# Westlake-AI/SemiReward

Measured on AMD Instinct MI355X. Metric: unlabeled images/sec/node (FlexMatch+SR, ViT-S CIFAR-100), higher is better.
Workload: dtype bf16

## Files before the change

### include/srhip.h

```cpp
#ifndef SRHIP_H
#define SRHIP_H

#ifdef __cplusplus
extern "C" {
#endif

enum {
  SRHIP_EPI_BF16 = 0,
  SRHIP_EPI_GELU_BF16 = 1,
  SRHIP_EPI_RESID_F32 = 2,
  SRHIP_EPI_DGELU_BF16 = 3,
  SRHIP_EPI_F32 = 4
};
int srhip_gemm_nt(int epilogue, const void* A, int lda, const void* B, int ldb, void* C, int ldc, int M, int N, int K,
                  const float* bias, const float* row_scale, int rows_per_sample, const void* aux_in, void* aux_out,
                  int ldaux, float alpha, float beta, void* stream);
#define SRHIP_GEMM_PLAN_TILE128 0
#define SRHIP_GEMM_PLAN_SMALL64 1
#define SRHIP_GEMM_PLAN_BIG256 2
#define SRHIP_GEMM_PLAN_BIG128 3
#define SRHIP_GEMM_PLAN_BIG2WG 4
#define SRHIP_GEMM_PLAN_PP256 5
int srhip_gemm_nt_plan(int epilogue, int M, int N, int K, float beta);
int srhip_gemm_nt_planned(int epilogue, const void* A, int lda, const void* B, int ldb, void* C, int ldc, int M, int N, int K,
// ... 22 lines not shown
#define SRHIP_TN_OVERWRITE 2
typedef struct srhip_group_tn_desc {
  const void* A; const void* B; float* C; float* dbias;
  int M, N, K, lda, ldb, ldc, tile_start, flags;
} srhip_group_tn_desc;
int srhip_gemm_tn_grouped_f32(const srhip_group_tn_desc* desc_dev, int n_problems, int total_tiles, float alpha, float beta,
                              void* stream);
typedef struct srhip_slab_desc {
  float* dst; const float* src; long long stride;
  int count, n_slabs, block_start, pad0;
} srhip_slab_desc;
int srhip_slab_reduce_f32(const srhip_slab_desc* desc_dev, int n, int total_blocks, void* stream);
int srhip_gemm_tn_grouped_pp_f32(const srhip_group_tn_desc* desc_dev, int n_problems, int total_tiles, float alpha, float beta,
                                 void* stream);

int srhip_attn_fwd(const void* qkv, void* out, float* lse, int B, int N, int H, float scale, void* stream);
int srhip_attn_bwd(const void* qkv, const void* out, const void* d_out, const float* lse, void* dqkv, float* delta_ws,
                   int B, int N, int H, float scale, void* stream);

int srhip_attn_masked_fwd(const void* qkv, void* out, float* lse, const int* key_len, int B, int N, int H, float scale,
                          unsigned drop_key, unsigned drop_thresh, float drop_scale, void* stream);
int srhip_attn_masked_bwd(const void* qkv, const void* out, const void* d_out, const float* lse, void* dqkv, float* delta_ws,
                          const int* key_len, int B, int N, int H, float scale, unsigned drop_key, unsigned drop_thresh,
                          float drop_scale, void* stream);

int srhip_layernorm_fwd(const float* x, const float* gamma, const float* beta, float eps, void* out, float* mean,
                        float* rstd, int M, int D, void* stream);
int srhip_layernorm_bwd(const void* dy, const float* x, const float* mean, const float* rstd, const float* gamma,
                        float* dx, float* dgamma, float* dbeta, int M, int D, void* stream);
int srhip_layernorm_bwd_cast(const void* dy, const float* x, const float* mean, const float* rstd, const float* gamma, float* dx, float* dgamma,
                             float* dbeta, void* out_bf16, const float* row_scale, int rows_per_sample, int M, int D, void* stream);
int srhip_layernorm_bwd_part(const void* dy, const float* x, const float* mean, const float* rstd, const float* gamma, float* dx, float* part,
                             int n_rep, void* out_bf16, const float* row_scale, int rows_per_sample, int M, int D, void* stream);
typedef struct srhip_ln_reduce_desc { float* dgamma; float* dbeta; } srhip_ln_reduce_desc;
int srhip_ln_grad_reduce(const srhip_ln_reduce_desc* desc_dev, float* part, int n_ln, int n_rep, int D, void* stream);
typedef struct srhip_dw_tail {
  const srhip_ln_reduce_desc* ln_desc; float* ln_part;
  const float* dlogits; const float* feat; float* dWh; float* dbh;
  const float* dx; const float* img; const int* img_index; float* dpos; float* dcls; float* pe_ws;
  int n_ln, n_rep, C, B, D, in_chans, HW, ps;
} srhip_dw_tail;
int srhip_gemm_tn_grouped_tail_f32(const srhip_group_tn_desc* desc_dev, int n_problems, int total_tiles, float alpha, float beta,
                                   const srhip_dw_tail* tail, void* stream);
int srhip_patch_embed_bwd_fold(const float* ws, float* dWp, float* dbp, int B, int C, int HW, int ps, int D, void* stream);

int srhip_mlp_fused(const float* x, float* x_out, const float* ln_gamma, const float* ln_beta, float eps, const void* W1,
                    const float* b1, const void* W2, const float* b2, const float* row_scale, int rows_per_sample, int save_rows,
                    void* save_ln2, void* save_pre, void* save_h, float* save_mean, float* save_rstd, int M, int D, int Hd,
                    void* stream);
int srhip_gelu_eval(const float* x, float* y_erf, float* y_poly, int n, void* stream);
int srhip_mlp_fused_proj(const float* x, float* x_out, const void* ao, const void* Wp, const float* bp, const float* row_scale1,
                         int ao_scaled, const float* ln_gamma, const float* ln_beta, float eps, const void* W1, const float* b1, const void* W2,
                         const float* b2, const float* row_scale2, int rows_per_sample, void* ln_next, const float* next_gamma,
                         const float* next_beta, int M, int D, int Hd, void* stream);

int srhip_attn_block_supported(int N, int D, int H);
int srhip_attn_block_fused(const void* xn_bf16, const void* Wqkv, const float* bqkv, const void* qkv_extra, void* out, const float* out_scale,
                           int B, int N, int D, int H, float scale, void* stream);

int srhip_patch_embed_fwd(const float* img, const int* img_index, const float* Wp, const float* bp, const float* cls,
                          const float* pos, float* x, int B, int C, int HW, int ps, int D, void* stream);
int srhip_patch_embed_bwd(const float* dx, const float* img, const int* img_index, float* dWp, float* dbp, float* dcls,
                          float* dpos, int B, int C, int HW, int ps, int D, void* stream);
long srhip_patch_embed_bwd_ws_floats(int B, int C, int HW, int ps, int D);
int srhip_patch_embed_bwd_ws(const float* dx, const float* img, const int* img_index, float* dWp, float* dbp, float* dcls,
                             float* dpos, float* ws, int B, int C, int HW, int ps, int D, void* stream);
// ... 272 lines not shown
```

### semireward_amd/_lib.py

```python
import ctypes
import os
from ctypes import c_double, c_float, c_int, c_long, c_longlong, c_uint, c_ulonglong, c_void_p

import torch

HERE = os.path.dirname(os.path.abspath(__file__))
LIB_PATH = os.path.join(HERE, "libsrhip.so")

EPI_BF16, EPI_GELU_BF16, EPI_RESID_F32, EPI_DGELU_BF16, EPI_F32 = range(5)
X3_EPI_F32, X3_EPI_GELU_F32, X3_EPI_RESID_F32 = range(3)
X3B_NT, X3B_NN = range(2)
X3B_EPI_F32, X3B_EPI_ACC, X3B_EPI_DGELU, X3B_EPI_GELU_PRE = range(4)
REDUCE_NONE, REDUCE_MEAN, REDUCE_SUM = range(3)

P, I, F, L, Dbl, U = c_void_p, c_int, c_float, c_long, c_double, c_uint
SIGNATURES = {
    "srhip_gemm_nt": (I, [I, P, I, P, I, P, I, I, I, I, P, P, I, P, P, I, F, F, P]),
    "srhip_gemm_nt_plan": (I, [I, I, I, I, F]),
    "srhip_gemm_nt_planned": (I, [I, P, I, P, I, P, I, I, I, I, P, P, I, P, P, I, F, F, I, P]),
    "srhip_vit_fork": (I, [P, P, P, I, I, I, I, P]),
    "srhip_vit_fanout": (I, [P, P, I, P, P, I, P, P, c_longlong, I, I, P]),
    "srhip_gemm_small_max_grid": (I, [I]),
    "srhip_gemm_nt_grouped_f32": (I, [P, I, I, F, F, P]),
    "srhip_gemm_nt_grouped_n64_f32": (I, [P, I, I, F, F, P]),
    "srhip_gemm_tn_grouped_f32": (I, [P, I, I, F, F, P]),
    "srhip_gemm_tn_grouped_pp_f32": (I, [P, I, I, F, F, P]),
    "srhip_gemm_tn_grouped_tail_f32": (I, [P, I, I, F, F, P, P]),
    "srhip_patch_embed_bwd_fold": (I, [P, P, P, I, I, I, I, I, P]),
    "srhip_slab_reduce_f32": (I, [P, I, I, P]),
    "srhip_attn_fwd": (I, [P, P, P, I, I, I, F, P]),
    "srhip_attn_bwd": (I, [P, P, P, P, P, P, I, I, I, F, P]),
    "srhip_layernorm_fwd": (I, [P, P, P, F, P, P, P, I, I, P]),
    "srhip_layernorm_bwd": (I, [P, P, P, P, P, P, P, P, I, I, P]),
    "srhip_layernorm_bwd_cast": (I, [P, P, P, P, P, P, P, P, P, P, I, I, I, P]),
    "srhip_layernorm_bwd_part": (I, [P, P, P, P, P, P, P, I, P, P, I, I, I, P]),
    "srhip_ln_grad_reduce": (I, [P, P, I, I, I, P]),
    "srhip_mlp_fused": (I, [P, P, P, P, F, P, P, P, P, P, I, I, P, P, P, P, P, I, I, I, P]),
    "srhip_attn_block_supported": (I, [I, I, I]),
    "srhip_attn_block_fused": (I, [P, P, P, P, P, P, I, I, I, I, F, P]),
    "srhip_gelu_eval": (I, [P, P, P, I, P]),
    "srhip_mlp_fused_proj": (I, [P, P, P, P, P, P, I, P, P, F, P, P, P, P, P, I, P, P, P, I, I, I, P]),
    "srhip_adam_bias_corrections": (I, [F, F, I, P]),
    "srhip_adamw_flat_dyn": (I, [P, P, P, P, P, P, P, I, P, P, P, F, F, F, Dbl, F, P, I, P]),
    "srhip_adam_flat_dyn": (I, [P, P, P, P, L, F, F, F, F, P, P]),
    "srhip_droppath_fill_cols_dyn": (I, [P, P, P, I, I, I, P, c_ulonglong, P]),
    "srhip_patch_embed_fwd": (I, [P, P, P, P, P, P, P, I, I, I, I, I, P]),
    "srhip_patch_embed_bwd": (I, [P, P, P, P, P, P, P, I, I, I, I, I, P]),
    "srhip_patch_embed_bwd_ws_floats": (L, [I, I, I, I, I]),
    "srhip_patch_embed_bwd_ws": (I, [P, P, P, P, P, P, P, P, I, I, I, I, I, P]),
    "srhip_patch_im2col": (I, [P, P, P, I, I, I, I, P]),
    "srhip_patch_assemble": (I, [P, P, P, P, P, I, I, I, P]),
    "srhip_patch_grad_operands": (I, [P, P, P, P, I, I, I, P]),
    "srhip_gemm_nt_x3": (I, [I, P, I, P, I, P, I, I, I, I, P, P, I, P]),
    "srhip_attn_fwd_x3": (I, [P, P, I, I, I, F, P]),
    "srhip_layernorm_fwd_f32": (I, [P, P, P, F, P, P, P, I, I, P]),
    "srhip_patch_im2col_f32": (I, [P, P, P, I, I, I, I, P]),
    "srhip_attn_fwd_x3_lse": (I, [P, P, P, I, I, I, F, P]),
    "srhip_gemm_x3": (I, [I, I, P, I, P, I, P, I, I, I, I, P, P, P, I, P]),
    "srhip_gemm_tn_x3_grouped": (I, [P, I, I, P]),
    "srhip_attn_bwd_x3": (I, [P, P, P, P, P, P, I, I, I, F, P]),
    "srhip_layernorm_bwd_part_f32": (I, [P, P, P, P, P, P, P, I, P, P, I, I, I, P]),
    "srhip_patch_grad_operands_f32": (I, [P, P, P, P, I, I, I, P]),
    "srhip_scale_rows_f32": (I, [P, P, I, P, L, I, P]),
    "srhip_cls_head_fwd": (I, [P, P, P, F, P, P, P, P, P, P, I, I, I, I, P]),
    "srhip_cls_head_fwd_scatter": (I, [P, P, P, F, P, P, P, P, P, P, P, P, P, I, I, I, I, P]),
    "srhip_cls_head_bwd": (I, [P, P, P, P, P, P, P, P, P, P, P, I, I, I, I, P]),
    "srhip_cast_scale_rows": (I, [P, P, I, P, L, I, P]),
    "srhip_transpose_to_bf16": (I, [P, I, I, P, I, I, I, I, I, P, P]),
# ... 136 lines not shown
```

### semireward_amd/csrc/vit_ops.hip

```cpp
#include "common.h"
#include "srhip.h"
#include "tail_ops.h"

namespace {

template <int NV, typename TOUT = bf16_t>
__global__ __launch_bounds__(256) void ln_fwd_kernel(const float* __restrict__ x, const float* __restrict__ gamma,
                                                    const float* __restrict__ beta, float eps, TOUT* __restrict__ out,
                                                    float* __restrict__ mean, float* __restrict__ rstd, int M) {
  constexpr int D = NV * 128, RW = 2;
  const int row0 = (blockIdx.x * 4 + (threadIdx.x >> 6)) * RW, lane = threadIdx.x & 63;
  if (row0 >= M) return;
  float2 v[RW][NV], g[NV], b[NV];
#pragma unroll
  for (int r = 0; r < RW; ++r) {
    const float2* xr = reinterpret_cast<const float2*>(x + (size_t)min(row0 + r, M - 1) * D);
#pragma unroll
    for (int i = 0; i < NV; ++i) v[r][i] = xr[i * 64 + lane];
  }
#pragma unroll
  for (int i = 0; i < NV; ++i) {
    g[i] = reinterpret_cast<const float2*>(gamma)[i * 64 + lane];
    b[i] = reinterpret_cast<const float2*>(beta)[i * 64 + lane];
  }
#pragma unroll
  for (int r = 0; r < RW; ++r) {
    const int row = row0 + r;
    if (row >= M) break;
    float s = 0.f;
#pragma unroll
    for (int i = 0; i < NV; ++i) s += v[r][i].x + v[r][i].y;
    const float mu = wave_sum(s) * (1.0f / D);
    float q = 0.f;
// ... 1 lines not shown
    for (int i = 0; i < NV; ++i) { const float a = v[r][i].x - mu, c = v[r][i].y - mu; q += a * a + c * c; }
    const float rs = rsqrtf(wave_sum(q) * (1.0f / D) + eps);
    if constexpr (sizeof(TOUT) == 4) {
      float2* orow = reinterpret_cast<float2*>(out + (size_t)row * D);
#pragma unroll
      for (int i = 0; i < NV; ++i)
        orow[i * 64 + lane] = make_float2((v[r][i].x - mu) * rs * g[i].x + b[i].x, (v[r][i].y - mu) * rs * g[i].y + b[i].y);
    } else {
      uint32_t* orow = reinterpret_cast<uint32_t*>(out + (size_t)row * D);
#pragma unroll
      for (int i = 0; i < NV; ++i)
        orow[i * 64 + lane] = pack_bf2((v[r][i].x - mu) * rs * g[i].x + b[i].x, (v[r][i].y - mu) * rs * g[i].y + b[i].y);
    }
    if (mean && lane == 0) { mean[row] = mu; rstd[row] = rs; }
  }
}

template <int NV, int RPW, typename TDY = bf16_t>
__global__ __launch_bounds__(256) void ln_bwd_kernel(const TDY* __restrict__ dy, const float* __restrict__ x,
                                                    const float* __restrict__ mean, const float* __restrict__ rstd,
                                                    const float* __restrict__ gamma, float* __restrict__ dx,
                                                    float* __restrict__ dgamma, float* __restrict__ dbeta, int M,
                                                    TDY* __restrict__ out_bf16, const float* __restrict__ row_scale, int rows_per_sample,
                                                    float* __restrict__ part, int n_rep) {
  constexpr int D = NV * 128;
  __shared__ float red[2][4][D];
  const int wave = threadIdx.x >> 6, lane = threadIdx.x & 63;
  float2 ag[NV], ab[NV], g[NV];
#pragma unroll
  for (int i = 0; i < NV; ++i) {
    ag[i] = make_float2(0.f, 0.f); ab[i] = make_float2(0.f, 0.f);
    g[i] = reinterpret_cast<const float2*>(gamma)[i * 64 + lane];
  }
  for (int rr = 0; rr < RPW; ++rr) {
    const int row = blockIdx.x * (4 * RPW) + wave * RPW + rr;
    if (row >= M) break;
    const float mu = mean[row], rs = rstd[row];
    const float2* xr = reinterpret_cast<const float2*>(x + (size_t)row * D);
    float2 xh[NV], gy[NV];
    float s1 = 0.f, s2 = 0.f;
#pragma unroll
    for (int i = 0; i < NV; ++i) {
      const float2 xv = xr[i * 64 + lane];
      float d0, d1;
      if constexpr (sizeof(TDY) == 4) {
        const float2 d2 = reinterpret_cast<const float2*>(dy + (size_t)row * D)[i * 64 + lane];
        d0 = d2.x; d1 = d2.y;
      } else {
        const uint32_t d2 = reinterpret_cast<const uint32_t*>(dy + (size_t)row * D)[i * 64 + lane];
        d0 = bf2f((bf16_t)(d2 & 0xffff)); d1 = bf2f((bf16_t)(d2 >> 16));
      }
      xh[i] = make_float2((xv.x - mu) * rs, (xv.y - mu) * rs);
      gy[i] = make_float2(d0 * g[i].x, d1 * g[i].y);
      s1 += gy[i].x + gy[i].y;
      s2 += gy[i].x * xh[i].x + gy[i].y * xh[i].y;
      ag[i].x += d0 * xh[i].x; ag[i].y += d1 * xh[i].y;
      ab[i].x += d0; ab[i].y += d1;
    }
    const float c1 = wave_sum(s1) * (1.0f / D), c2 = wave_sum(s2) * (1.0f / D);
    float2* dxr = reinterpret_cast<float2*>(dx + (size_t)row * D);
#pragma unroll
    for (int i = 0; i < NV; ++i) {
      float2 o = dxr[i * 64 + lane];
      o.x += rs * (gy[i].x - c1 - xh[i].x * c2);
      o.y += rs * (gy[i].y - c1 - xh[i].y * c2);
      dxr[i * 64 + lane] = o;
      if (out_bf16) {
        const float sc = row_scale ? row_scale[row / rows_per_sample] : 1.0f;
        if constexpr (sizeof(TDY) == 4) reinterpret_cast<float2*>(out_bf16 + (size_t)row * D)[i * 64 + lane] = make_float2(o.x * sc, o.y * sc);
        else reinterpret_cast<uint32_t*>(out_bf16 + (size_t)row * D)[i * 64 + lane] = pack_bf2(o.x * sc, o.y * sc);
      }
    }
  }
  if (n_rep > 0) { dgamma = part + (size_t)(blockIdx.x % n_rep) * 2 * D; dbeta = dgamma + D; }
  if (!dgamma) return;
#pragma unroll
  for (int i = 0; i < NV; ++i) {
    const int c = (i * 64 + lane) * 2;
    red[0][wave][c] = ag[i].x; red[0][wave][c + 1] = ag[i].y;
    red[1][wave][c] = ab[i].x; red[1][wave][c + 1] = ab[i].y;
  }
  __syncthreads();
  for (int c = threadIdx.x; c < D; c += 256) {
    atomicAdd(dgamma + c, red[0][0][c] + red[0][1][c] + red[0][2][c] + red[0][3][c]);
    atomicAdd(dbeta + c, red[1][0][c] + red[1][1][c] + red[1][2][c] + red[1][3][c]);
  }
}

__global__ void patch_embed_fwd_kernel(const float* __restrict__ img, const int* __restrict__ img_index,
                                       const float* __restrict__ Wp, const float* __restrict__ bp,
                                       const float* __restrict__ cls, const float* __restrict__ pos,
                                       float* __restrict__ x, int C, int HW, int ps, int D) {
  extern __shared__ __attribute__((aligned(16))) float patch[];
  const int gw = HW / ps, N = gw * gw + 1, K = C * ps * ps;
  const int b = blockIdx.y, t0 = blockIdx.x * PE_TOK, d = threadIdx.x;
  const int bi = img_index ? img_index[b] : b;
  const float* im = img + (size_t)bi * C * HW * HW;
  for (int e = threadIdx.x; e < PE_TOK * K; e += blockDim.x) {
    const int tt = e / K, k = e % K, t = t0 + tt;
    float v = 0.f;
    if (t >= 1 && t < N) {
      const int p = t - 1, py = p / gw, px = p % gw;
      const int c = k / (ps * ps), i = (k / ps) % ps, j = k % ps;
      v = im[((size_t)c * HW + py * ps + i) * HW + px * ps + j];
    }
// ... 645 lines not shown
```

### semireward_amd/nets/vit.py

```python
import math
import types

import numpy as np
import torch

from .. import ops
from .pretrained import load_checkpoint
from .surface import ModuleSurface


class VitConfig:
    def __init__(self, img_size=224, patch_size=16, in_chans=3, num_classes=1000, embed_dim=768, depth=12,
                 num_heads=12, mlp_ratio=4.0, drop_path_rate=0.0, eps=1e-6):
        self.img_size, self.patch_size, self.in_chans, self.num_classes = img_size, patch_size, in_chans, num_classes
        self.embed_dim, self.depth, self.num_heads, self.mlp_ratio = embed_dim, depth, num_heads, mlp_ratio
        self.drop_path_rate, self.eps = drop_path_rate, eps
        assert embed_dim % num_heads == 0 and embed_dim // num_heads == 64, "libsrhip attention is built for head_dim 64"
        assert embed_dim in (128, 384, 768)

    @property
    def num_tokens(self):
        return (self.img_size // self.patch_size) ** 2 + 1

    @property
    def hidden(self):
        return int(self.embed_dim * self.mlp_ratio)


def param_names_shapes(cfg):
    D, Hd, p, C = cfg.embed_dim, cfg.hidden, cfg.patch_size, cfg.num_classes
    out = [("cls_token", (1, 1, D)), ("pos_embed", (1, cfg.num_tokens, D)),
           ("patch_embed.proj.weight", (D, cfg.in_chans, p, p)), ("patch_embed.proj.bias", (D,))]
    for i in range(cfg.depth):
        b = "blocks.%d." % i
        out += [(b + "norm1.weight", (D,)), (b + "norm1.bias", (D,)),
                (b + "attn.qkv.weight", (3 * D, D)), (b + "attn.qkv.bias", (3 * D,)),
                (b + "attn.proj.weight", (D, D)), (b + "attn.proj.bias", (D,)),
                (b + "norm2.weight", (D,)), (b + "norm2.bias", (D,)),
                (b + "mlp.fc1.weight", (Hd, D)), (b + "mlp.fc1.bias", (Hd,)),
                (b + "mlp.fc2.weight", (D, Hd)), (b + "mlp.fc2.bias", (D,))]
    out += [("norm.weight", (D,)), ("norm.bias", (D,)), ("head.weight", (C, D)), ("head.bias", (C,))]
    return out


DW_GROUPS = 3
LN_REP = 16
_FUSED_MLP = True
_FUSED_ATTN = True
_FUSED_PROJ = True
_FUSED_NEXT_LN = True
_FUSED_MLP_MIN_ROWS = 16384


def _fused_mlp(cfg, rows):
    Hd = cfg.hidden
    return cfg.embed_dim == 384 and Hd % 128 == 0 and Hd <= 4096 and rows >= _FUSED_MLP_MIN_ROWS and _FUSED_MLP


def launch_kernels(cfg, n_images, kernels_as_images=None, precision="bf16"):
    if precision == "bf16x3":
        return ("bf16x3",)
    D, N, H, Hd = cfg.embed_dim, cfg.num_tokens, cfg.num_heads, cfg.hidden
    M = n_images * N
    fused = _fused_mlp(cfg, max(M, (kernels_as_images or 0) * N))
    fused_attn = _FUSED_ATTN and ops.attn_block_supported(N, D, H)
    gemms = []
    if cfg.in_chans * cfg.patch_size ** 2 > 64:
        gemms.append((ops.EPI_F32, n_images * (N - 1), D, cfg.in_chans * cfg.patch_size ** 2))
    if not fused_attn:
        gemms.append((ops.EPI_BF16, M, 3 * D, D))
    if not (fused and _FUSED_PROJ):
        gemms.append((ops.EPI_RESID_F32, M, D, D))
    if not fused:
        gemms += [(ops.EPI_GELU_BF16, M, Hd, D), (ops.EPI_RESID_F32, M, D, Hd)]
    return (fused, fused_attn) + tuple(ops.gemm_nt_plan(e, m, n, k) for e, m, n, k in gemms)


def droppath_keep_host(probs, depth, B, seed, cols=None):
    p = np.asarray(probs, dtype=np.float32)[:depth]
    col = np.arange(B, dtype=np.int64) if cols is None else np.asarray(cols, dtype=np.int64)
    col = np.where((col < 0) | (col >= B), 0, col)
    i = (np.arange(2 * depth, dtype=np.int64)[:, None] * B + col[None, :]).astype(np.uint64)
    with np.errstate(over="ignore"):
# ... 386 lines not shown
                g2=r(Ti["g2"]), dpre=r(Ti["dpre"]), g1=r(Ti["g1"]), dqkv=r(Ti["dqkv"]), pre=r(ctx.pre[i]), xmid=r(ctx.xmid[i]), xs=r(ctx.xs[i]),
                st1=(r(ctx.st1[i][0]), r(ctx.st1[i][1])), st2=(r(ctx.st2[i][0]), r(ctx.st2[i][1])), qkv=r(ctx.qkv[i]), ao=r(ctx.ao[i]),
                lse=im(ctx.lse[i])))
        self._buf_cache[key] = v
        return v

    def backward_rows(self, ctx, dlogits, b0, b1):
        cfg = self.cfg
        D, N, H, Hd, C = cfg.embed_dim, cfg.num_tokens, cfg.num_heads, cfg.hidden, cfg.num_classes
        nb = b1 - b0
        M = nb * N
        P = self.p
        G = lambda n: self.p(n, self.grad)
        x3 = ctx.precision == "bf16x3"
        if x3:
            ln_bwd, attn_bwd, NN, X3F = ops.layernorm_bwd_part_f32, ops.attn_bwd_x3, ops.X3B_NN, ops.X3B_EPI_F32
        else:
            ln_bwd, attn_bwd, wT = ops.layernorm_bwd_part, ops.attn_bwd, self.wT
            self.ensure_transposed()
        T = self._bwd_plan(ctx.B * N, ctx)
        v = self._bwd_views(ctx, T, b0, b1)
        dl = dlogits if (b0 == 0 and b1 == ctx.B) else dlogits[b0:b1]
        v.dx.zero_()
        ops.cls_head_bwd(dl, P("head.weight"), P("norm.weight"), None, v.xhat, v.rstd, v.dx, None, None, G("norm.weight"), G("norm.bias"),
                         nb, N, D, C)
        scale = 64 ** -0.5
        dp = ctx.dp
        lnp = T["ln_part"]
        cb = self.grad_ready_cb if (b0 == 0 and b1 == ctx.B and not x3) else None
        self._groups_launched = cb is not None
        gdone = {g["lo_layer"]: g for g in T["groups"]} if cb is not None else {}
        dpr = (lambda i_, j_: ops.RawRows(dp, i_ * dp.stride(0) + j_ * dp.stride(1) + b0)) if dp is not None else (lambda i_, j_: None)
        L = v.layers
        (ops.scale_rows_f32 if x3 else ops.cast_scale_rows)(v.dx, dpr(cfg.depth - 1, 1), N, L[cfg.depth - 1].g2, M, D)
        for i in reversed(range(cfg.depth)):
            b = "blocks.%d." % i
            Li = L[i]
            s1 = dpr(i, 0)
            if x3:
                ops.gemm_x3(NN, ops.X3B_EPI_DGELU, Li.g2, P(b + "mlp.fc2.weight"), Li.dpre, M, Hd, D, aux=Li.pre, ldaux=Hd)
                ops.gemm_x3(NN, X3F, Li.dpre, P(b + "mlp.fc1.weight"), v.dln, M, D, Hd)
            else:
                ops.gemm_nt(ops.EPI_DGELU_BF16, Li.g2, wT[b + "mlp.fc2.weight"], Li.dpre, M, Hd, D, aux_in=Li.pre, ldaux=Hd)
                ops.gemm_nt(ops.EPI_BF16, Li.dpre, wT[b + "mlp.fc1.weight"], v.dln, M, D, Hd)
            ln_bwd(v.dln, Li.xmid, Li.st2[0], Li.st2[1], P(b + "norm2.weight"), v.dx, lnp[2 * i + 1], LN_REP, Li.g1, s1, N, M, D)
            if x3:
                ops.gemm_x3(NN, X3F, Li.g1, P(b + "attn.proj.weight"), v.dao, M, D, D)
            else:
                ops.gemm_nt(ops.EPI_BF16, Li.g1, wT[b + "attn.proj.weight"], v.dao, M, D, D)
            attn_bwd(Li.qkv, Li.ao, v.dao, Li.lse, Li.dqkv, v.delta, nb, N, H, scale)
            if x3:
                ops.gemm_x3(NN, X3F, Li.dqkv, P(b + "attn.qkv.weight"), v.dln, M, D, 3 * D)
            else:
                ops.gemm_nt(ops.EPI_BF16, Li.dqkv, wT[b + "attn.qkv.weight"], v.dln, M, D, 3 * D)
            ln_bwd(v.dln, Li.xs, Li.st1[0], Li.st1[1], P(b + "norm1.weight"), v.dx, lnp[2 * i], LN_REP,
                   L[i - 1].g2 if i > 0 else None, dpr(i - 1, 1) if i > 0 else None, N, M, D)
            g = gdone.get(i)
            if g is not None:
                desc, npb, ntiles, flops, nbytes = g["desc"]
                ops.gemm_tn_grouped_f32(desc, npb, ntiles, alpha=1.0, beta=1.0, flops=flops, nbytes=nbytes)
                ops.ln_grad_reduce(g["ln_desc"], lnp[2 * g["lo_layer"]:2 * g["hi_layer"]], 2 * (g["hi_layer"] - g["lo_layer"]), LN_REP, D)
                cb(*g["flat"])

    def backward_finish(self, ctx, dlogits):
        cfg = self.cfg
        D, N, C = cfg.embed_dim, cfg.num_tokens, cfg.num_classes
        B = ctx.B
        M = B * N
        f32 = torch.float32
        G = lambda n: self.p(n, self.grad)
        x3 = ctx.precision == "bf16x3"
        T = self._bwd_plan(M, ctx)
        dx = self._buf("b3_dx" if x3 else "b_dx", (M, D), f32)
        small_pe = cfg.in_chans * cfg.patch_size ** 2 <= 64
        ws = self._buf("b_pe_ws", (ops.patch_embed_bwd_ws_floats(B, cfg.in_chans, cfg.img_size, cfg.patch_size, D),), f32) if small_pe else None
        groups_launched = not x3 and getattr(self, "_groups_launched", False)
        merged = not x3 and not groups_launched and ops._PROFILE is None and getattr(T["desc"][0], "reduce", None) is None
        desc, npb, ntiles, flops, nbytes = T["desc"]
        if merged:
            pe = (dx, ctx.img, ctx.img_index, G("pos_embed"), G("cls_token"), ws, B, cfg.in_chans, cfg.img_size, cfg.patch_size) if small_pe else None
            ops.gemm_tn_grouped_tail_f32(desc, npb, ntiles, D, ln=(T["ln_desc"], T["ln_part"], 2 * cfg.depth, LN_REP),
                                         head=(dlogits, ctx.feat, G("head.weight"), G("head.bias"), B, C), pe=pe)
        else:
            ops.cls_head_bwd(dlogits, None, None, ctx.feat, None, None, None, G("head.weight"), G("head.bias"), None, None, B, N, D, C)
            if not groups_launched:
                ops.ln_grad_reduce(T["ln_desc"], T["ln_part"], 2 * cfg.depth, LN_REP, D)
                if x3:
                    ops.gemm_tn_x3_grouped(desc, npb, ntiles, flops=flops, nbytes=nbytes)
                else:
# ... 62 lines not shown
```

### semireward_amd/ops.py

```python
import ctypes
import os

import torch

from . import _lib
from ._lib import EPI_BF16, EPI_DGELU_BF16, EPI_F32, EPI_GELU_BF16, EPI_RESID_F32
from ._lib import X3_EPI_F32, X3_EPI_GELU_F32, X3_EPI_RESID_F32
from ._lib import X3B_NT, X3B_NN, X3B_EPI_F32, X3B_EPI_ACC, X3B_EPI_DGELU, X3B_EPI_GELU_PRE
from ._lib import REDUCE_NONE, REDUCE_MEAN, REDUCE_SUM


_CHECK_ARGS = os.environ.get("SRHIP_CHECK_ARGS", "0") != "0"


def _p_checked(t):
    if t is None:
        return None
    assert t.is_cuda and t.is_contiguous(), "libsrhip needs contiguous device tensors"
    return t.data_ptr()


def _p_fast(t):
    return None if t is None else t.data_ptr()

# ... 161 lines not shown

def gemm_nt(epi, A, B, C, M, N, K, *, lda=None, ldb=None, ldc=None, bias=None, row_scale=None, rows_per_sample=0,
            aux_in=None, aux_out=None, ldaux=0, alpha=1.0, beta=0.0, plan_M=None):
    if plan_M is not None:
        args = (epi, _p(A), lda or K, _p(B), ldb or K, _p(C), ldc or N, M, N, K, _p(bias), _p(row_scale), rows_per_sample, _p(aux_in),
                _p(aux_out), ldaux, alpha, beta, int(plan_M), _s())
        if _PROFILE is not None:
            _PROFILE.timed("srhip_gemm_nt_planned", args, 2.0 * M * N * K, _GemmProfile.kernel_name(epi, int(plan_M), N, K),
                           _GemmProfile.gemm_bytes(epi, M, N, K, aux_in, aux_out, beta))
            return
        _call("srhip_gemm_nt_planned", *args)
        return
    if _PROFILE is not None:
        _PROFILE.timed("srhip_gemm_nt", (epi, _p(A), lda or K, _p(B), ldb or K, _p(C), ldc or N, M, N, K, _p(bias), _p(row_scale),
              rows_per_sample, _p(aux_in), _p(aux_out), ldaux, alpha, beta, _s(),), 2.0 * M * N * K, _GemmProfile.kernel_name(epi, M, N, K),
                              _GemmProfile.gemm_bytes(epi, M, N, K, aux_in, aux_out, beta))
        return
    _call("srhip_gemm_nt", epi, _p(A), lda or K, _p(B), ldb or K, _p(C), ldc or N, M, N, K, _p(bias), _p(row_scale),
          rows_per_sample, _p(aux_in), _p(aux_out), ldaux, alpha, beta, _s())


GEMM_PLAN_NAMES = {0: "tile128", 1: "small64", 2: "big256", 3: "big128", 4: "big2wg", 5: "pp256"}


def gemm_nt_plan(epi, M, N, K, beta=0.0):
    rc = int(_lib.lib().srhip_gemm_nt_plan(epi, M, N, K, beta))
    if rc < 0:
        _lib.check(rc, "srhip_gemm_nt_plan")
    return GEMM_PLAN_NAMES[rc]


GEMM_SMALL_ALONE, GEMM_SMALL_CONTENDED = 256, 40
_small_max_grid = None


def gemm_small_max_grid(n):
    global _small_max_grid
    if n != _small_max_grid:
        _lib.lib().srhip_gemm_small_max_grid(int(n))
        _small_max_grid = n


GROUP_DESC_DTYPE = [("A", "<u8"), ("B", "<u8"), ("C", "<u8"), ("M", "<i4"), ("N", "<i4"), ("K", "<i4"), ("lda", "<i4"),
                    ("ldb", "<i4"), ("ldc", "<i4"), ("tile_start", "<i4"), ("pad0", "<i4"), ("pad1", "<i4"), ("pad2", "<i4")]


def make_group_desc(problems, device):
    import numpy as np
    arr = np.zeros(len(problems), dtype=GROUP_DESC_DTYPE)
    t = 0
    for i, (A, B, C, M, N, K) in enumerate(problems):
        arr[i] = (_p(A), _p(B), _p(C), M, N, K, K, K, N, t, 0, 0, 0)
        t += ((M + 127) // 128) * ((N + 127) // 128)
    assert arr.itemsize == 64
    flops = float(sum(2.0 * M * N * K for _, _, _, M, N, K in problems))
    nbytes = float(sum(2.0 * (M * K + N * K) + 8.0 * M * N for _, _, _, M, N, K in problems))
    return torch.from_numpy(arr.view(np.uint8).copy()).to(device), len(problems), t, flops, nbytes


def gemm_nt_grouped_f32(desc, n_problems, total_tiles, alpha=1.0, beta=1.0, flops=0.0, nbytes=0.0, n64=False):
    fn, kern = ("srhip_gemm_nt_grouped_n64_f32", "gemm_grouped_n64_f32_kernel") if n64 else ("srhip_gemm_nt_grouped_f32", "gemm_grouped_f32_kernel")
    if _PROFILE is not None:
        _PROFILE.timed(fn, (_p(desc), n_problems, total_tiles, alpha, beta, _s(),), flops, kern, nbytes)
        return
    _call(fn, _p(desc), n_problems, total_tiles, alpha, beta, _s())

# ... 174 lines not shown
    if _PROFILE is not None:
        M = B * N
        _PROFILE.timed("srhip_attn_block_fused", (_p(xn), _p(Wqkv), _p(bqkv), _p(qkv_extra), _p(out), _p(out_scale), B, N, D, H, scale, _s(),), 2.0 * M * 3 * D * D + 4.0 * B * H * N * N * 64, "attn_block_kernel<%d>" % N,
                              2.0 * M * D + 2.0 * M * D + 2.0 * 3 * D * D)
        return
    _call("srhip_attn_block_fused", _p(xn), _p(Wqkv), _p(bqkv), _p(qkv_extra), _p(out), _p(out_scale), B, N, D, H, scale, _s())


def attn_fwd(qkv, out, lse, B, N, H, scale):
    if _PROFILE is not None:
        _PROFILE.timed("srhip_attn_fwd", (_p(qkv), _p(out), _p(lse), B, N, H, scale, _s()), 4.0 * B * H * N * N * 64, "attn_fwd_kernel",
                       2.0 * B * N * 4 * H * 64)
        return
    _call("srhip_attn_fwd", _p(qkv), _p(out), _p(lse), B, N, H, scale, _s())


def attn_bwd(qkv, out, d_out, lse, dqkv, delta_ws, B, N, H, scale):
    if _PROFILE is not None:
        _PROFILE.timed("srhip_attn_bwd", (_p(qkv), _p(out), _p(d_out), _p(lse), _p(dqkv), _p(delta_ws), B, N, H, scale, _s()),
                       10.0 * B * H * N * N * 64, "attn_bwd (dq + dkv kernels)", 2.0 * B * N * 8 * H * 64)
        return
    _call("srhip_attn_bwd", _p(qkv), _p(out), _p(d_out), _p(lse), _p(dqkv), _p(delta_ws), B, N, H, scale, _s())


def layernorm_fwd(x, gamma, beta, eps, out, mean, rstd, M, D):
    _call("srhip_layernorm_fwd", _p(x), _p(gamma), _p(beta), eps, _p(out), _p(mean), _p(rstd), M, D, _s())


def layernorm_bwd_cast(dy, x, mean, rstd, gamma, dx, dgamma, dbeta, out_bf16, row_scale, rows_per_sample, M, D):
    _call("srhip_layernorm_bwd_cast", _p(dy), _p(x), _p(mean), _p(rstd), _p(gamma), _p(dx), _p(dgamma), _p(dbeta), _p(out_bf16), _p(row_scale),
          rows_per_sample, M, D, _s())


def layernorm_bwd_part(dy, x, mean, rstd, gamma, dx, part, n_rep, out_bf16, row_scale, rows_per_sample, M, D):
    if _PROFILE is not None:
        _PROFILE.timed("srhip_layernorm_bwd_part", (_p(dy), _p(x), _p(mean), _p(rstd), _p(gamma), _p(dx), _p(part), n_rep, _p(out_bf16),
                                                    _p(row_scale), rows_per_sample, M, D, _s()), 0.0, "ln_bwd_kernel", 16.0 * M * D)
        return
    _call("srhip_layernorm_bwd_part", _p(dy), _p(x), _p(mean), _p(rstd), _p(gamma), _p(dx), _p(part), n_rep, _p(out_bf16), _p(row_scale),
          rows_per_sample, M, D, _s())


def make_ln_reduce_desc(pairs, device):
    import numpy as np
    arr = np.array([[_p(g), _p(b)] for g, b in pairs], dtype=np.uint64)
    desc = torch.from_numpy(arr.view(np.uint8).copy()).to(device)
    desc.out_ranges = [(_p(t), t.numel() * t.element_size()) for pair in pairs for t in pair]
    return desc


def ln_grad_reduce(desc, part, n_ln, n_rep, D):
    _call("srhip_ln_grad_reduce", _p(desc), _p(part), n_ln, n_rep, D, _s())


def mlp_fused(x, gamma, beta, eps, W1, b1, W2, b2, row_scale, rows_per_sample, M, D, Hd, x_out=None, save=None):
    rows, ln2, pre, h, mean, rstd = save if save is not None else (0, None, None, None, None, None)
    args = (_p(x), _p(x_out if x_out is not None else x), _p(gamma), _p(beta), eps, _p(W1), _p(b1), _p(W2), _p(b2), _p(row_scale),
            rows_per_sample, rows, _p(ln2), _p(pre), _p(h), _p(mean), _p(rstd), M, D, Hd)
    if _PROFILE is not None:
        _PROFILE.timed("srhip_mlp_fused", (*args, _s(),), 4.0 * M * D * Hd, "mlp_fused_kernel<384, 0, 4>",
                              8.0 * M * D + 4.0 * D * Hd + rows * (2.0 * D + 4.0 * Hd))
        return
    _call("srhip_mlp_fused", *args, _s())


def mlp_fused_proj(x, ao, Wp, bp, row_scale1, gamma, beta, eps, W1, b1, W2, b2, row_scale2, rows_per_sample, M, D, Hd, x_out=None,
                   ln_next=None, next_gamma=None, next_beta=None, ao_scaled=False):
# ... 848 lines not shown
```

Measured before the change: 1634.

## Fuse LayerNorm backward with the following proj/fc2 NT GEMM in ViT backward

Adds a kernel that runs the LayerNorm backward for a 32-row block, keeps the resulting bf16 gradient rows in LDS, and then immediately runs the consuming NT GEMM (attn.proj, or the previous layer's fc2 with a deferred dGELU epilogue) from those on-chip rows while streaming B tiles in via buffer-load-to-LDS. The ViT backward uses it for proj always and for fc2 when the small-GEMM grid is contended, which saves a kernel launch and a global round-trip of the LN output. In exchange, each block holds a large LDS footprint and only M/32 blocks run, which can limit occupancy and GEMM efficiency compared with the standalone tuned GEMM. The LN row code is also factored into a shared header.

```diff
diff --git a/include/srhip.h b/include/srhip.h
--- a/include/srhip.h
+++ b/include/srhip.h
@@ -78,6 +78,9 @@
                              float* dbeta, void* out_bf16, const float* row_scale, int rows_per_sample, int M, int D, void* stream);
 int srhip_layernorm_bwd_part(const void* dy, const float* x, const float* mean, const float* rstd, const float* gamma, float* dx, float* part,
                              int n_rep, void* out_bf16, const float* row_scale, int rows_per_sample, int M, int D, void* stream);
+int srhip_layernorm_bwd_part_gemm(const void* dy, const float* x, const float* mean, const float* rstd, const float* gamma, float* dx, float* part,
+                                  int n_rep, void* out_bf16, const float* row_scale, int rows_per_sample, int M, int D, const void* B, int ldb,
+                                  void* C, int ldc, int N, int epilogue, const void* aux_in, int ldaux, void* stream);
 typedef struct srhip_ln_reduce_desc { float* dgamma; float* dbeta; } srhip_ln_reduce_desc;
 int srhip_ln_grad_reduce(const srhip_ln_reduce_desc* desc_dev, float* part, int n_ln, int n_rep, int D, void* stream);
 typedef struct srhip_dw_tail {
diff --git a/semireward_amd/_lib.py b/semireward_amd/_lib.py
--- a/semireward_amd/_lib.py
+++ b/semireward_amd/_lib.py
@@ -34,6 +34,7 @@
     "srhip_layernorm_bwd": (I, [P, P, P, P, P, P, P, P, I, I, P]),
     "srhip_layernorm_bwd_cast": (I, [P, P, P, P, P, P, P, P, P, P, I, I, I, P]),
     "srhip_layernorm_bwd_part": (I, [P, P, P, P, P, P, P, I, P, P, I, I, I, P]),
+    "srhip_layernorm_bwd_part_gemm": (I, [P, P, P, P, P, P, P, I, P, P, I, I, I, P, I, P, I, I, I, P, I, P]),
     "srhip_ln_grad_reduce": (I, [P, P, I, I, I, P]),
     "srhip_mlp_fused": (I, [P, P, P, P, F, P, P, P, P, P, I, I, P, P, P, P, P, I, I, I, P]),
     "srhip_attn_block_supported": (I, [I, I, I]),
diff --git a/semireward_amd/csrc/ln_bwd_gemm.hip b/semireward_amd/csrc/ln_bwd_gemm.hip
--- /dev/null
+++ b/semireward_amd/csrc/ln_bwd_gemm.hip
@@ -0,0 +1,238 @@
+#include "common.h"
+#include "ln_bwd_row.h"
+#include "srhip.h"
+
+namespace {
+
+constexpr int LD = 384, NV = 3, BK = 32, KS = LD / BK;
+constexpr int CN = 128;
+constexpr int TILE_EL = CN * BK;
+constexpr int GS = 2, NG = KS / GS;
+
+__device__ __forceinline__ int swz(int row) { return (0x78 >> (((row >> 2) & 3) * 2)) & 3; }
+
+typedef __attribute__((address_space(3))) void lds_void;
+template <int N_>
+__device__ __forceinline__ void wait_vm() { asm volatile("s_waitcnt vmcnt(%0)" ::"n"(N_) : "memory"); }
+
+struct LnGemmArgs {
+  const bf16_t* dy;
+  const float *x, *mean, *rstd, *gamma;
+  float *dx, *part;
+  bf16_t* out;
+  const float* row_scale;
+  const bf16_t* B;
+  bf16_t* C;
+  const bf16_t* aux_in;
+  int M, N, n_rep, rows_per_sample, ldb, ldc, ldaux;
+};
+
+template <int R, int EPI>
+__global__ __launch_bounds__(512) void ln_bwd_then_nt_kernel(LnGemmArgs a) {
+  constexpr int RPW = R / 8, NB = RPW / 4;
+  constexpr int WN = 256 / R, NTW = CN / WN / 16;
+  constexpr int A_EL = R * LD;
+  static_assert(R % 32 == 0 && RPW % 4 == 0 && 2 * 8 * NB * LD * 4 <= A_EL * 2, "layout");
+  __shared__ __attribute__((aligned(16))) bf16_t sm[A_EL + KS * TILE_EL];
+  const int tid = threadIdx.x, lane = tid & 63;
+  const int wave = __builtin_amdgcn_readfirstlane(tid >> 6);
+  const int l15 = lane & 15, lg = lane >> 4;
+  const int m0 = blockIdx.x * R;
+  const int nchunk = a.N / CN;
+
+  const int pr = 16 * wave + (lane >> 2);
+  const int lo = (pr * a.ldb + (((lane & 3) ^ swz(pr)) << 3)) * 2;
+  const __amdgpu_buffer_rsrc_t rb = __builtin_amdgcn_make_buffer_rsrc(const_cast<bf16_t*>(a.B), 0, a.N * a.ldb * 2, 0x00020000);
+  constexpr int OOB = 0x7ffffff0;
+  auto issue = [&](int c, int kt) {
+    lds_void* dst = (lds_void*)(sm + A_EL + kt * TILE_EL + 16 * wave * BK);
+    __builtin_amdgcn_raw_ptr_buffer_load_lds(rb, dst, 16, c < nchunk ? lo : OOB, (c * CN * a.ldb + kt * BK) * 2, 0, 0);
+  };
+#pragma unroll
+  for (int p = 0; p < (NG - 1) * GS; ++p) issue(0, p);
+
+  float2 ag[NB][NV], ab[NB][NV], g[NV];
+#pragma unroll
+  for (int i = 0; i < NV; ++i) {
+#pragma unroll
+    for (int b = 0; b < NB; ++b) { ag[b][i] = make_float2(0.f, 0.f); ab[b][i] = make_float2(0.f, 0.f); }
+    g[i] = reinterpret_cast<const float2*>(a.gamma)[i * 64 + lane];
+  }
+  const int wslot = (lane & 15) >> 2, win = 2 * (lane & 3);
+#pragma unroll
+  for (int rb4 = 0; rb4 < RPW; rb4 += 4) {
+    LnBwdRow<NV, bf16_t, true> rw[4];
+    const int r0 = wave * RPW + rb4;
+#pragma unroll
+    for (int j = 0; j < 4; ++j)
+      ln_bwd_row_load(rw[j], a.dy, a.x, a.mean, a.rstd, a.dx, a.row_scale, a.rows_per_sample, min(m0 + r0 + j, a.M - 1), lane);
+#pragma unroll
+    for (int j = 0; j < 4; ++j) {
+      const int r = r0 + j;
+      if (m0 + r >= a.M) break;
+      bf16_t* arow = sm + r * BK + ((wslot ^ swz(r)) << 3) + win;
+      ln_bwd_row_apply(rw[j], g, ag[rb4 / 4], ab[rb4 / 4], a.dx, a.out, a.row_scale, a.rows_per_sample, m0 + r, lane, [&](int i, uint32_t pk) {
+        *reinterpret_cast<uint32_t*>(arow + ((i * 64 + lane) >> 4) * (R * BK)) = pk;
+      });
+    }
+  }
+  wait_vm<0>();
+  __syncthreads();
+
+  const int wm = wave / WN, wn = wave % WN;
+  s16x8_t fb[2][KS];
+#pragma unroll
+  for (int mt = 0; mt < 2; ++mt) {
+    const int rm = wm * 32 + mt * 16 + l15;
+#pragma unroll
+    for (int kt = 0; kt < KS; ++kt) fb[mt][kt] = *reinterpret_cast<const s16x8_t*>(sm + kt * (R * BK) + rm * BK + ((lg ^ swz(rm)) << 3));
+  }
+  __syncthreads();
+
+  {
+    constexpr int NP = 8 * NB;
+    float* red = reinterpret_cast<float*>(sm);
+#pragma unroll
+    for (int b = 0; b < NB; ++b)
+#pragma unroll
+      for (int i = 0; i < NV; ++i) {
+        const int c = (i * 64 + lane) * 2;
+        *reinterpret_cast<float2*>(red + (wave * NB + b) * LD + c) = ag[b][i];
+        *reinterpret_cast<float2*>(red + (NP + wave * NB + b) * LD + c) = ab[b][i];
+      }
+    __syncthreads();
+    float* dst = a.part + (size_t)(blockIdx.x % a.n_rep) * 2 * LD;
+    for (int c = tid; c < 2 * LD; c += 512) {
+      const float* p = red + (c >= LD ? NP * LD + c - LD : c);
+      float t[NP];
+#pragma unroll
+      for (int w = 0; w < NP; ++w) t[w] = p[w * LD];
+#pragma unroll
+      for (int st = 1; st < NP; st <<= 1)
+#pragma unroll
+        for (int w = 0; w < NP; w += 2 * st) t[w] += t[w + st];
+      atomicAdd(dst + c, t[0]);
+    }
+  }
+
+  int fo_a[NTW];
+#pragma unroll
+  for (int t = 0; t < NTW; ++t) { const int rn = wn * (16 * NTW) + t * 16 + l15; fo_a[t] = A_EL + rn * BK + ((lg ^ swz(rn)) << 3); }
+  int mrow[2];
+#pragma unroll
+  for (int mt = 0; mt < 2; ++mt) mrow[mt] = m0 + wm * 32 + mt * 16 + l15;
+  constexpr bool DEFER = EPI == SRHIP_EPI_DGELU_BF16;
+  constexpr int NE = NTW * 2 * 4;
+  f32x4_t accp[NTW][2];
+  u32x2_t auxp[NTW][2];
+  float ev[NTW][2][4];
+  int n0p = 0;
+  auto epi_elem = [&](int e) __attribute__((always_inline)) {
+    const int nt = e >> 3, mt = (e >> 2) & 1, r = e & 3;
+    const uint32_t p = auxp[nt][mt][r >> 1];
+    ev[nt][mt][r] = accp[nt][mt][r] * gelu_erf_grad(bf2f((bf16_t)((r & 1) ? (p >> 16) : (p & 0xffff))));
+    if (r == 3 && mrow[mt] < a.M)
+      *reinterpret_cast<u32x2_t*>(a.C + (size_t)mrow[mt] * a.ldc + n0p + nt * 16) =
+          u32x2_t{pack_bf2(ev[nt][mt][0], ev[nt][mt][1]), pack_bf2(ev[nt][mt][2], ev[nt][mt][3])};
+  };
+  auto chunk = [&](auto prev_c, int c) __attribute__((always_inline)) {
+    constexpr bool PREV = decltype(prev_c)::value;
+    const int n0 = c * CN + wn * (16 * NTW) + lg * 4;
+    f32x4_t acc[NTW][2];
+    u32x2_t aux[NTW][2];
+#pragma unroll
+    for (int nt = 0; nt < NTW; ++nt)
+#pragma unroll
+      for (int mt = 0; mt < 2; ++mt) acc[nt][mt] = f32x4_t{0.f, 0.f, 0.f, 0.f};
+#pragma unroll
+    for (int j = 0; j < NG; ++j) {
+      wait_vm<(NG - 2) * GS>();
+      __builtin_amdgcn_s_barrier();
+#pragma unroll
+      for (int i = 0; i < GS; ++i) {
+        const int s = (j + NG - 1) * GS + i;
+        issue(c + s / KS, s % KS);
+      }
+      if (DEFER && j == 0) {
+#pragma unroll
+        for (int nt = 0; nt < NTW; ++nt)
+#pragma unroll
+          for (int mt = 0; mt < 2; ++mt)
+            aux[nt][mt] = *reinterpret_cast<const u32x2_t*>(a.aux_in + (size_t)min(mrow[mt], a.M - 1) * a.ldaux + n0 + nt * 16);
+      }
+#pragma unroll
+      for (int i = 0; i < GS; ++i) {
+        const int kt = j * GS + i;
+        s16x8_t fa[NTW];
+#pragma unroll
+        for (int nt = 0; nt < NTW; ++nt) fa[nt] = *reinterpret_cast<const s16x8_t*>(sm + kt * TILE_EL + fo_a[nt]);
+#pragma unroll
+        for (int nt = 0; nt < NTW; ++nt)
+#pragma unroll
+          for (int mt = 0; mt < 2; ++mt)
+            acc[nt][mt] = __builtin_amdgcn_mfma_f32_16x16x32_bf16(__builtin_bit_cast(bf16x8_t, fa[nt]), __builtin_bit_cast(bf16x8_t, fb[mt][kt]),
+                                                                  acc[nt][mt], 0, 0, 0);
+        if constexpr (DEFER && PREV) {
+#pragma unroll
+          for (int e = (kt * NE) / KS; e < ((kt + 1) * NE) / KS; ++e) epi_elem(e);
+        }
+      }
+    }
+    if constexpr (DEFER) {
+#pragma unroll
+      for (int nt = 0; nt < NTW; ++nt)
+#pragma unroll
+        for (int mt = 0; mt < 2; ++mt) { accp[nt][mt] = acc[nt][mt]; auxp[nt][mt] = aux[nt][mt]; }
+      n0p = n0;
+    } else {
+#pragma unroll
+      for (int mt = 0; mt < 2; ++mt) {
+        if (mrow[mt] >= a.M) continue;
+#pragma unroll
+        for (int nt = 0; nt < NTW; ++nt)
+          *reinterpret_cast<u32x2_t*>(a.C + (size_t)mrow[mt] * a.ldc + n0 + nt * 16) =
+              u32x2_t{pack_bf2(acc[nt][mt][0], acc[nt][mt][1]), pack_bf2(acc[nt][mt][2], acc[nt][mt][3])};
+      }
+    }
+  };
+  chunk(std::false_type{}, 0);
+  for (int c = 1; c < nchunk; ++c) chunk(std::true_type{}, c);
+  if constexpr (DEFER) {
+#pragma unroll
+    for (int e = 0; e < NE; ++e) epi_elem(e);
+  }
+  wait_vm<0>();
+}
+
+#ifndef SRHIP_LNB_ROWS
+#define SRHIP_LNB_ROWS 32
+#endif
+constexpr int ROWS = SRHIP_LNB_ROWS;
+
+}
+
+extern "C" int srhip_layernorm_bwd_part_gemm(const void* dy, const float* x, const float* mean, const float* rstd, const float* gamma, float* dx,
+                                             float* part, int n_rep, void* out_bf16, const float* row_scale, int rows_per_sample, int M, int D,
+                                             const void* B, int ldb, void* C, int ldc, int N, int epilogue, const void* aux_in, int ldaux,
+                                             void* stream) {
+  auto al = [](const void* p, uintptr_t n) { return ((uintptr_t)p & (n - 1)) == 0; };
+  if (M <= 0 || D != LD || N <= 0 || N % CN != 0 || !dy || !x || !mean || !rstd || !gamma || !dx || !part || n_rep <= 0 || !out_bf16 || !B || !C)
+    return SR_EINVAL;
+  if (row_scale && rows_per_sample <= 0) return SR_EINVAL;
+  if (epilogue != SRHIP_EPI_BF16 && epilogue != SRHIP_EPI_DGELU_BF16) return SR_EINVAL;
+  if (ldb < LD || ldb % 8 != 0 || ldc < N || ldc % 4 != 0 || (long long)N * ldb * 2 >= 0x7ffffff0LL) return SR_EINVAL;
+  if (epilogue == SRHIP_EPI_DGELU_BF16 && (!aux_in || ldaux < N || ldaux % 4 != 0 || !al(aux_in, 8))) return SR_EINVAL;
+  if (!al(dy, 4) || !al(x, 8) || !al(dx, 8) || !al(out_bf16, 4) || !al(gamma, 8) || !al(part, 4) || !al(mean, 4) || !al(rstd, 4) ||
+      (row_scale && !al(row_scale, 4)) || !al(B, 16) || !al(C, 8))
+    return SR_EINVAL;
+  LnGemmArgs a;
+  a.dy = (const bf16_t*)dy; a.x = x; a.mean = mean; a.rstd = rstd; a.gamma = gamma; a.dx = dx; a.part = part; a.out = (bf16_t*)out_bf16;
+  a.row_scale = row_scale; a.B = (const bf16_t*)B; a.C = (bf16_t*)C; a.aux_in = (const bf16_t*)aux_in;
+  a.M = M; a.N = N; a.n_rep = n_rep; a.rows_per_sample = rows_per_sample > 0 ? rows_per_sample : 1; a.ldb = ldb; a.ldc = ldc; a.ldaux = ldaux;
+  hipStream_t s = (hipStream_t)stream;
+  const dim3 grid(cdiv(M, ROWS)), block(512);
+  if (epilogue == SRHIP_EPI_BF16) SR_LAUNCH((ln_bwd_then_nt_kernel<ROWS, SRHIP_EPI_BF16>), grid, block, 0, s, a);
+  else SR_LAUNCH((ln_bwd_then_nt_kernel<ROWS, SRHIP_EPI_DGELU_BF16>), grid, block, 0, s, a);
+  SR_CHECK_LAUNCH();
+  return SR_OK;
+}
diff --git a/semireward_amd/csrc/ln_bwd_row.h b/semireward_amd/csrc/ln_bwd_row.h
--- /dev/null
+++ b/semireward_amd/csrc/ln_bwd_row.h
@@ -0,0 +1,76 @@
+#pragma once
+#include "common.h"
+
+template <int NV, typename TDY, bool PRE = false>
+struct LnBwdRow {
+  float2 xv[NV];
+  float2 o[PRE ? NV : 1];
+  typename std::conditional<sizeof(TDY) == 4, float2, uint32_t>::type d[NV];
+  float mu, rs, sc;
+};
+
+template <int NV, typename TDY, bool PRE>
+__device__ __forceinline__ void ln_bwd_row_load(LnBwdRow<NV, TDY, PRE>& r, const TDY* __restrict__ dy, const float* __restrict__ x,
+                                                const float* __restrict__ mean, const float* __restrict__ rstd, const float* dx,
+                                                const float* __restrict__ row_scale, int rows_per_sample, int row, int lane) {
+  constexpr int D = NV * 128;
+  r.mu = mean[row]; r.rs = rstd[row];
+  if constexpr (PRE) r.sc = row_scale ? row_scale[row / rows_per_sample] : 1.0f;
+  const float2* xr = reinterpret_cast<const float2*>(x + (size_t)row * D);
+  const float2* dxr = reinterpret_cast<const float2*>(dx + (size_t)row * D);
+#pragma unroll
+  for (int i = 0; i < NV; ++i) {
+    r.xv[i] = xr[i * 64 + lane];
+    if constexpr (sizeof(TDY) == 4) r.d[i] = reinterpret_cast<const float2*>(dy + (size_t)row * D)[i * 64 + lane];
+    else r.d[i] = reinterpret_cast<const uint32_t*>(dy + (size_t)row * D)[i * 64 + lane];
+    if constexpr (PRE) r.o[i] = dxr[i * 64 + lane];
+  }
+}
+
+template <int NV, typename TDY, bool PRE, typename KEEP>
+__device__ __forceinline__ void ln_bwd_row_apply(const LnBwdRow<NV, TDY, PRE>& r, const float2 (&g)[NV], float2 (&ag)[NV], float2 (&ab)[NV],
+                                                 float* __restrict__ dx, TDY* __restrict__ out, const float* __restrict__ row_scale,
+                                                 int rows_per_sample, int row, int lane, KEEP&& keep) {
+  constexpr int D = NV * 128;
+  const float mu = r.mu, rs = r.rs;
+  float2 xh[NV], gy[NV];
+  float s1 = 0.f, s2 = 0.f;
+#pragma unroll
+  for (int i = 0; i < NV; ++i) {
+    const float2 xv = r.xv[i];
+    float d0, d1;
+    if constexpr (sizeof(TDY) == 4) {
+      d0 = r.d[i].x; d1 = r.d[i].y;
+    } else {
+      const uint32_t d2 = r.d[i];
+      d0 = bf2f((bf16_t)(d2 & 0xffff)); d1 = bf2f((bf16_t)(d2 >> 16));
+    }
+    xh[i] = make_float2((xv.x - mu) * rs, (xv.y - mu) * rs);
+    gy[i] = make_float2(d0 * g[i].x, d1 * g[i].y);
+    s1 += gy[i].x + gy[i].y;
+    s2 += gy[i].x * xh[i].x + gy[i].y * xh[i].y;
+    ag[i].x += d0 * xh[i].x; ag[i].y += d1 * xh[i].y;
+    ab[i].x += d0; ab[i].y += d1;
+  }
+  const float c1 = wave_sum(s1) * (1.0f / D), c2 = wave_sum(s2) * (1.0f / D);
+  float2* dxr = reinterpret_cast<float2*>(dx + (size_t)row * D);
+#pragma unroll
+  for (int i = 0; i < NV; ++i) {
+    float2 o;
+    if constexpr (PRE) o = r.o[i]; else o = dxr[i * 64 + lane];
+    o.x += rs * (gy[i].x - c1 - xh[i].x * c2);
+    o.y += rs * (gy[i].y - c1 - xh[i].y * c2);
+    dxr[i * 64 + lane] = o;
+    if (out) {
+      float sc;
+      if constexpr (PRE) sc = r.sc; else sc = row_scale ? row_scale[row / rows_per_sample] : 1.0f;
+      if constexpr (sizeof(TDY) == 4) {
+        reinterpret_cast<float2*>(out + (size_t)row * D)[i * 64 + lane] = make_float2(o.x * sc, o.y * sc);
+      } else {
+        const uint32_t pk = pack_bf2(o.x * sc, o.y * sc);
+        reinterpret_cast<uint32_t*>(out + (size_t)row * D)[i * 64 + lane] = pk;
+        keep(i, pk);
+      }
+    }
+  }
+}
diff --git a/semireward_amd/csrc/vit_ops.hip b/semireward_amd/csrc/vit_ops.hip
--- a/semireward_amd/csrc/vit_ops.hip
+++ b/semireward_amd/csrc/vit_ops.hip
@@ -1,4 +1,5 @@
 #include "common.h"
+#include "ln_bwd_row.h"
 #include "srhip.h"
 #include "tail_ops.h"
 
@@ -66,45 +67,14 @@
     ag[i] = make_float2(0.f, 0.f); ab[i] = make_float2(0.f, 0.f);
     g[i] = reinterpret_cast<const float2*>(gamma)[i * 64 + lane];
   }
+  constexpr int UNR = (RPW == 2 || NV == 3) ? RPW : 1;
+#pragma unroll UNR
   for (int rr = 0; rr < RPW; ++rr) {
     const int row = blockIdx.x * (4 * RPW) + wave * RPW + rr;
     if (row >= M) break;
-    const float mu = mean[row], rs = rstd[row];
-    const float2* xr = reinterpret_cast<const float2*>(x + (size_t)row * D);
-    float2 xh[NV], gy[NV];
-    float s1 = 0.f, s2 = 0.f;
-#pragma unroll
-    for (int i = 0; i < NV; ++i) {
-      const float2 xv = xr[i * 64 + lane];
-      float d0, d1;
-      if constexpr (sizeof(TDY) == 4) {
-        const float2 d2 = reinterpret_cast<const float2*>(dy + (size_t)row * D)[i * 64 + lane];
-        d0 = d2.x; d1 = d2.y;
-      } else {
-        const uint32_t d2 = reinterpret_cast<const uint32_t*>(dy + (size_t)row * D)[i * 64 + lane];
-        d0 = bf2f((bf16_t)(d2 & 0xffff)); d1 = bf2f((bf16_t)(d2 >> 16));
-      }
-      xh[i] = make_float2((xv.x - mu) * rs, (xv.y - mu) * rs);
-      gy[i] = make_float2(d0 * g[i].x, d1 * g[i].y);
-      s1 += gy[i].x + gy[i].y;
-      s2 += gy[i].x * xh[i].x + gy[i].y * xh[i].y;
-      ag[i].x += d0 * xh[i].x; ag[i].y += d1 * xh[i].y;
-      ab[i].x += d0; ab[i].y += d1;
-    }
-    const float c1 = wave_sum(s1) * (1.0f / D), c2 = wave_sum(s2) * (1.0f / D);
-    float2* dxr = reinterpret_cast<float2*>(dx + (size_t)row * D);
-#pragma unroll
-    for (int i = 0; i < NV; ++i) {
-      float2 o = dxr[i * 64 + lane];
-      o.x += rs * (gy[i].x - c1 - xh[i].x * c2);
-      o.y += rs * (gy[i].y - c1 - xh[i].y * c2);
-      dxr[i * 64 + lane] = o;
-      if (out_bf16) {
-        const float sc = row_scale ? row_scale[row / rows_per_sample] : 1.0f;
-        if constexpr (sizeof(TDY) == 4) reinterpret_cast<float2*>(out_bf16 + (size_t)row * D)[i * 64 + lane] = make_float2(o.x * sc, o.y * sc);
-        else reinterpret_cast<uint32_t*>(out_bf16 + (size_t)row * D)[i * 64 + lane] = pack_bf2(o.x * sc, o.y * sc);
-      }
-    }
+    LnBwdRow<NV, TDY> r;
+    ln_bwd_row_load(r, dy, x, mean, rstd, dx, row_scale, rows_per_sample, row, lane);
+    ln_bwd_row_apply(r, g, ag, ab, dx, out_bf16, row_scale, rows_per_sample, row, lane, [](int, uint32_t) {});
   }
   if (n_rep > 0) { dgamma = part + (size_t)(blockIdx.x % n_rep) * 2 * D; dbeta = dgamma + D; }
   if (!dgamma) return;
diff --git a/semireward_amd/nets/vit.py b/semireward_amd/nets/vit.py
--- a/semireward_amd/nets/vit.py
+++ b/semireward_amd/nets/vit.py
@@ -1,4 +1,5 @@
 import math
+import os
 import types
 
 import numpy as np
@@ -49,6 +50,7 @@
 _FUSED_ATTN = True
 _FUSED_PROJ = True
 _FUSED_NEXT_LN = True
+_FUSED_LN_BWD = os.environ.get("SRHIP_FUSED_LN_BWD", "auto")
 _FUSED_MLP_MIN_ROWS = 16384
 
 
@@ -501,6 +503,10 @@
         gdone = {g["lo_layer"]: g for g in T["groups"]} if cb is not None else {}
         dpr = (lambda i_, j_: ops.RawRows(dp, i_ * dp.stride(0) + j_ * dp.stride(1) + b0)) if dp is not None else (lambda i_, j_: None)
         L = v.layers
+        fuse = 0
+        if not x3 and D == 384 and Hd % 128 == 0 and cb is None:
+            fuse = (2 if ops.small_max_grid_is_contended() else 1) if _FUSED_LN_BWD == "auto" else int(_FUSED_LN_BWD)
+        fuse_proj, fuse_fc2 = fuse >= 1, fuse >= 2
         (ops.scale_rows_f32 if x3 else ops.cast_scale_rows)(v.dx, dpr(cfg.depth - 1, 1), N, L[cfg.depth - 1].g2, M, D)
         for i in reversed(range(cfg.depth)):
             b = "blocks.%d." % i
@@ -510,20 +516,29 @@
                 ops.gemm_x3(NN, ops.X3B_EPI_DGELU, Li.g2, P(b + "mlp.fc2.weight"), Li.dpre, M, Hd, D, aux=Li.pre, ldaux=Hd)
                 ops.gemm_x3(NN, X3F, Li.dpre, P(b + "mlp.fc1.weight"), v.dln, M, D, Hd)
             else:
-                ops.gemm_nt(ops.EPI_DGELU_BF16, Li.g2, wT[b + "mlp.fc2.weight"], Li.dpre, M, Hd, D, aux_in=Li.pre, ldaux=Hd)
+                if not fuse_fc2 or i == cfg.depth - 1:
+                    ops.gemm_nt(ops.EPI_DGELU_BF16, Li.g2, wT[b + "mlp.fc2.weight"], Li.dpre, M, Hd, D, aux_in=Li.pre, ldaux=Hd)
                 ops.gemm_nt(ops.EPI_BF16, Li.dpre, wT[b + "mlp.fc1.weight"], v.dln, M, D, Hd)
-            ln_bwd(v.dln, Li.xmid, Li.st2[0], Li.st2[1], P(b + "norm2.weight"), v.dx, lnp[2 * i + 1], LN_REP, Li.g1, s1, N, M, D)
-            if x3:
-                ops.gemm_x3(NN, X3F, Li.g1, P(b + "attn.proj.weight"), v.dao, M, D, D)
-            else:
-                ops.gemm_nt(ops.EPI_BF16, Li.g1, wT[b + "attn.proj.weight"], v.dao, M, D, D)
+            if fuse_proj:
+                ln_bwd(v.dln, Li.xmid, Li.st2[0], Li.st2[1], P(b + "norm2.weight"), v.dx, lnp[2 * i + 1], LN_REP, Li.g1, s1, N, M, D,
+                       (wT[b + "attn.proj.weight"], v.dao, D, ops.EPI_BF16, None, 0))
+            else:
+                ln_bwd(v.dln, Li.xmid, Li.st2[0], Li.st2[1], P(b + "norm2.weight"), v.dx, lnp[2 * i + 1], LN_REP, Li.g1, s1, N, M, D)
+                if x3:
+                    ops.gemm_x3(NN, X3F, Li.g1, P(b + "attn.proj.weight"), v.dao, M, D, D)
+                else:
+                    ops.gemm_nt(ops.EPI_BF16, Li.g1, wT[b + "attn.proj.weight"], v.dao, M, D, D)
             attn_bwd(Li.qkv, Li.ao, v.dao, Li.lse, Li.dqkv, v.delta, nb, N, H, scale)
             if x3:
                 ops.gemm_x3(NN, X3F, Li.dqkv, P(b + "attn.qkv.weight"), v.dln, M, D, 3 * D)
             else:
                 ops.gemm_nt(ops.EPI_BF16, Li.dqkv, wT[b + "attn.qkv.weight"], v.dln, M, D, 3 * D)
-            ln_bwd(v.dln, Li.xs, Li.st1[0], Li.st1[1], P(b + "norm1.weight"), v.dx, lnp[2 * i], LN_REP,
-                   L[i - 1].g2 if i > 0 else None, dpr(i - 1, 1) if i > 0 else None, N, M, D)
+            if fuse_fc2 and i > 0:
+                ln_bwd(v.dln, Li.xs, Li.st1[0], Li.st1[1], P(b + "norm1.weight"), v.dx, lnp[2 * i], LN_REP, L[i - 1].g2, dpr(i - 1, 1), N, M, D,
+                       (wT["blocks.%d.mlp.fc2.weight" % (i - 1)], L[i - 1].dpre, Hd, ops.EPI_DGELU_BF16, L[i - 1].pre, Hd))
+            else:
+                ln_bwd(v.dln, Li.xs, Li.st1[0], Li.st1[1], P(b + "norm1.weight"), v.dx, lnp[2 * i], LN_REP,
+                       L[i - 1].g2 if i > 0 else None, dpr(i - 1, 1) if i > 0 else None, N, M, D)
             g = gdone.get(i)
             if g is not None:
                 desc, npb, ntiles, flops, nbytes = g["desc"]
diff --git a/semireward_amd/ops.py b/semireward_amd/ops.py
--- a/semireward_amd/ops.py
+++ b/semireward_amd/ops.py
@@ -217,6 +217,10 @@
 
 GEMM_SMALL_ALONE, GEMM_SMALL_CONTENDED = 256, 40
 _small_max_grid = None
+
+
+def small_max_grid_is_contended():
+    return _small_max_grid == GEMM_SMALL_CONTENDED
 
 
 def gemm_small_max_grid(n):
@@ -457,7 +461,18 @@
           rows_per_sample, M, D, _s())
 
 
-def layernorm_bwd_part(dy, x, mean, rstd, gamma, dx, part, n_rep, out_bf16, row_scale, rows_per_sample, M, D):
+def layernorm_bwd_part(dy, x, mean, rstd, gamma, dx, part, n_rep, out_bf16, row_scale, rows_per_sample, M, D, then=None):
+    if then is not None:
+        B, C, N, epi, aux_in, ldaux = then[:6]
+        if len(then) > 6 and then[6] is not None:
+            _lib.check(-1, "srhip_layernorm_bwd_part_gemm")
+        if _PROFILE is not None:
+            layernorm_bwd_part(dy, x, mean, rstd, gamma, dx, part, n_rep, out_bf16, row_scale, rows_per_sample, M, D)
+            gemm_nt(epi, out_bf16, B, C, M, N, D, aux_in=aux_in, ldaux=ldaux)
+            return
+        _call("srhip_layernorm_bwd_part_gemm", _p(dy), _p(x), _p(mean), _p(rstd), _p(gamma), _p(dx), _p(part), n_rep, _p(out_bf16),
+              _p(row_scale), rows_per_sample, M, D, _p(B), D, _p(C), N, N, epi, _p(aux_in), ldaux, _s())
+        return
     if _PROFILE is not None:
         _PROFILE.timed("srhip_layernorm_bwd_part", (_p(dy), _p(x), _p(mean), _p(rstd), _p(gamma), _p(dx), _p(part), n_rep, _p(out_bf16),
                                                     _p(row_scale), rows_per_sample, M, D, _s()), 0.0, "ln_bwd_kernel", 16.0 * M * D)
```

New measurement: 1631. No clear change (-0.2%).
